# DhruvDh/highway-rope-ppo

Hardware: AMD Instinct MI355X
Metric: env-steps/sec (rollout+PPO update), 4096 envs × 15 vehicles, 1/2/4/8 GPUs (higher is better)
Workload: dtype fp32; 1 GPU; configs[1]: 4096 lockstep envs/GPU x 51 simulated vehicles, 15 observed x 4 features, sorted, no PE; PPO h256, 8 epochs x 32 minibatches (batch_size 64 -> 2048/64), rollout 32 steps/env; order=sorted, pe=none, obs_vehicles=15, envs_per_gpu=4096, global_envs=4096, rollout_len=32, samples_per_update=131072, hidden_dim=256, epochs=8, minibatches_per_epoch=32, parallelism=env-sharded dp1, library_build_flags=0

## Files before the change

### highway-rope-ppo_amd/csrc/ppo_kernels.hip

```cpp
#include <hip/hip_runtime.h>
#include <stdint.h>
#include <stdlib.h>
#include <string.h>

#include <algorithm>
#include <cmath>
#include <type_traits>

#include "hwy_ppo.h"

typedef float f32x16 __attribute__((ext_vector_type(16)));

#if defined(HWY_SECTION_PROFILE) || defined(HWY_CLOCK_PROBE)
__device__ unsigned long long g_ppo_sections[16];
#endif
#ifdef HWY_CLOCK_PROBE
__device__ unsigned long long g_ppo_wgt[2][1024][3];
#define CLK_BEGIN                                         \
  const uint64_t _c0 = __builtin_amdgcn_s_memtime();      \
  const uint64_t _r0 = __builtin_amdgcn_s_memrealtime();
#define CLK_END(k)                                                                   \
  do {                                                                               \
    if (threadIdx.x == 0) {                                                          \
      const uint64_t _r1 = __builtin_amdgcn_s_memrealtime();                         \
// ... 1139 lines not shown
    row_epi_bias_relu(acc, bias[0], H1, PH, nb);
  __syncthreads();
  if (h1g) rows_out<NT, RT>(H1, PH, h1g + (long)row0 * H, H, H, nrows);
  PSEC(1);
  zero_acc(acc);
  R.template run<1>(H1, PH, acc);
  if constexpr (MSK)
    mb[1] = row_epi_bias_relu_bits(acc, bias[1], H2, PH, nb);
  else
    row_epi_bias_relu(acc, bias[1], H2, PH, nb);
  __syncthreads();
  if (h2g) rows_out<NT, RT>(H2, PH, h2g + (long)row0 * H, H, H, nrows);
  PSEC(2);
  if constexpr (KEEP) {
    zero_acc(av);
    R.template run<2>(H2, PH, av);
    bias_relu_regs(av, bias[2]);
    zero_acc(cv);
    R.template run<3>(H2, PH, cv);
    bias_relu_regs(cv, bias[3]);
    return;
  }
  zero_acc(acc);
  R.template run<2>(H2, PH, acc);
  row_epi_bias_relu(acc, bias[2], AC, PA, nb);
  zero_acc(acc);
  R.template run<3>(H2, PH, acc);
  row_epi_bias_relu(acc, bias[3], AC + H, PA, nb);
  __syncthreads();
}

__device__ __forceinline__ float squash_corr(float z) {
  return log1pf(-(tanhf(z) * tanhf(z)) + 1e-6f);
}

template <int QH, int NW, int RT, bool CMP, bool WIDE = false>
__device__ __forceinline__ void rows_body(const RowArgs& r) {
  constexpr int H = 64 * QH;
  constexpr int TW = H / NW / 16;
  constexpr int RB = RT / 16;
  constexpr int RPW = RT / NW;
  constexpr int NT = 64 * NW;
  static_assert(TW * 16 * NW == H, "H must split into 16-column tiles per wave");
  static_assert(RT % 16 == 0 && RPW >= 1 && RPW <= 16, "RT: whole 16-row blocks, <= 16 head rows per wave");
  constexpr int PH = lds_pitch(H), PA = lds_pitch(2 * H), PXMAX = lds_pitch(kMaxRowS);
  constexpr bool kOwnX = !CMP && PXMAX > PA;
  static_assert(!CMP || (PA <= 2 * PH && PXMAX <= PH), "CMP: dac spans P0 | P1, the states fit P1");
  __shared__ __attribute__((aligned(16))) float XX[kOwnX ? RT * PXMAX : 4];
  __shared__ __attribute__((aligned(16))) float H1[CMP ? 2 * RT * PH : RT * PH];
  __shared__ __attribute__((aligned(16))) float H2[CMP ? 4 : RT * PH];
  __shared__ __attribute__((aligned(16))) float ACI[CMP ? 4 : RT * PA];
  float* const P1 = CMP ? H1 + RT * PH : H2;
  float* const AC = CMP ? H1 : ACI;
  __shared__ __attribute__((aligned(16))) f32x4 HDOT[NW][RT];
  __shared__ __attribute__((aligned(16))) f32x4 HROW[RT];
  __shared__ float HTAIL[NW][12];
#include "ppo_rows_body.inc"
}

template <int QH, int NW, int RT>
constexpr int rows_lds_floats() {
  constexpr int H = 64 * QH, PH = lds_pitch(H), PA = lds_pitch(2 * H), PXMAX = lds_pitch(kMaxRowS);
  return (PXMAX > PA ? RT * PXMAX : 0) + 2 * RT * PH + RT * PA + 4 * NW * RT + 4 * RT + 12 * NW;
}

template <int QH, int NW, int RT, bool WIDE = false>
__device__ __forceinline__ void rows_body_dyn(const RowArgs& r, float* arena) {
  constexpr bool CMP = false;
  constexpr int H = 64 * QH;
  constexpr int TW = H / NW / 16;
  constexpr int RB = RT / 16;
  constexpr int RPW = RT / NW;
  constexpr int NT = 64 * NW;
  static_assert(TW * 16 * NW == H && RT % 16 == 0 && RPW >= 1 && RPW <= 16, "rows_body's geometry");
  constexpr int PH = lds_pitch(H), PA = lds_pitch(2 * H), PXMAX = lds_pitch(kMaxRowS);
  constexpr bool kOwnX = PXMAX > PA;
  constexpr int oH1 = kOwnX ? RT * PXMAX : 0, oH2 = oH1 + RT * PH, oAC = oH2 + RT * PH;
  constexpr int oHD = oAC + RT * PA, oHR = oHD + 4 * NW * RT, oHT = oHR + 4 * RT;
  static_assert(oHT + 12 * NW == rows_lds_floats<QH, NW, RT>(), "arena layout");
  float* const XX = arena;
  float* const H1 = arena + oH1;
  float* const H2 = arena + oH2;
  float* const ACI = arena + oAC;
  float* const P1 = H2;
  float* const AC = ACI;
  f32x4(*const HDOT)[RT] = reinterpret_cast<f32x4(*)[RT]>(arena + oHD);
  f32x4* const HROW = reinterpret_cast<f32x4*>(arena + oHR);
  float(*const HTAIL)[12] = reinterpret_cast<float(*)[12]>(arena + oHT);
#include "ppo_rows_body.inc"
}

template <int QH, int NW, int RT>
__global__ void __launch_bounds__(64 * NW, 1) ppo_rows(RowArgs r) {
  rows_body<QH, NW, RT, false>(r);
}

template <int QH, int NW, int RT>
__global__ void __launch_bounds__(64 * NW) __attribute__((amdgpu_waves_per_eu(2 * NW / 4, 8)))
ppo_rows_c(RowArgs r) {
  CLK_BEGIN
  rows_body<QH, NW, RT, true>(r);
  CLK_END(0);
}

template <int QH, int NW>
__global__ void __launch_bounds__(64 * NW) __attribute__((amdgpu_waves_per_eu(NW / 4, 8)))
ppo_rows_c64(RowArgs r) {
  CLK_BEGIN
  rows_body<QH, NW, 64, true>(r);
  CLK_END(0);
}

struct ActArgs {
  int B, S;
  const float* states;
  const float* params;
  int64_t off[13];
  const float* noise;
  float *action, *pre_tanh, *logp, *value;
  const float* tiles;
#ifdef HWY_PPO_VMASK_TU
  const uint8_t *vm_trunc, *vm_term;
#endif
};

#ifdef HWY_PPO_VMASK_TU
__device__ __forceinline__ uint64_t vmask_tile(const ActArgs& r, int row0, int nrows, int lane) {
  bool mk = false;
  if (lane < nrows) {
    const long b = row0 + lane;
    mk = r.vm_trunc[b] != 0 && !(r.vm_term && r.vm_term[b] != 0);
  }
  return __ballot(mk);
}
#endif

template <int QH, int NW, bool TL, bool WIDE = false>
__device__ __forceinline__ void act_body(ActArgs r) {
  constexpr int H = 64 * QH;
  constexpr int RPW = kRowTile / NW;
  constexpr int PH = lds_pitch(H), PA = lds_pitch(2 * H), PXMAX = lds_pitch(kMaxRowS);
  __shared__ __attribute__((aligned(16))) float X[kRowTile * PXMAX];
  __shared__ __attribute__((aligned(16))) float H1[kRowTile * PH];
  __shared__ __attribute__((aligned(16))) float H2[kRowTile * PH];
  __shared__ __attribute__((aligned(16))) float AC[kRowTile * PA];
#include "ppo_act_body.inc"
}

template <int QH>
constexpr int act_lds_floats() {
  return kRowTile * (lds_pitch(kMaxRowS) + 2 * lds_pitch(64 * QH) + lds_pitch(128 * QH));
}
template <int QH, int NW, int RT>
constexpr int act_c_lds_floats() { return 2 * RT * lds_pitch(64 * QH) + 4 * NW * RT; }

template <int QH, int NW, bool TL, bool WIDE = false>
__device__ __forceinline__ void act_body_dyn(ActArgs r, float* arena) {
  constexpr int H = 64 * QH;
  constexpr int RPW = kRowTile / NW;
  constexpr int PH = lds_pitch(H), PA = lds_pitch(2 * H), PXMAX = lds_pitch(kMaxRowS);
  static_assert(kRowTile * (PXMAX + 2 * PH + PA) == act_lds_floats<QH>(), "arena layout");
  float* const X = arena;
  float* const H1 = arena + kRowTile * PXMAX;
  float* const H2 = arena + kRowTile * (PXMAX + PH);
  float* const AC = arena + kRowTile * (PXMAX + 2 * PH);
#include "ppo_act_body.inc"
}

template <int QH, int NW, bool TL>
__global__ void __launch_bounds__(64 * NW, 1) ppo_act(ActArgs r) {
  act_body<QH, NW, TL>(r);
}

template <int QH, int NW, int RT, bool WIDE = false>
__device__ __forceinline__ void act_c_body(ActArgs r) {
  constexpr int H = 64 * QH;
  constexpr int TW = H / NW / 16;
  constexpr int RB = RT / 16;
  constexpr int RPW = RT / NW;
  constexpr int PH = lds_pitch(H), PXMAX = lds_pitch(kMaxRowS);
  static_assert(TW * 16 * NW == H && PXMAX <= PH && RPW >= 1 && RPW <= 16, "ppo_act_c geometry");
  __shared__ __attribute__((aligned(16))) float P01[2 * RT * PH];
  __shared__ __attribute__((aligned(16))) f32x4 HDOT[NW][RT];
#include "ppo_act_c_body.inc"
}

template <int QH, int NW, int RT, bool WIDE = false>
__device__ __forceinline__ void act_c_body_dyn(ActArgs r, float* arena) {
  constexpr int H = 64 * QH;
  constexpr int TW = H / NW / 16;
  constexpr int RB = RT / 16;
  constexpr int RPW = RT / NW;
  constexpr int PH = lds_pitch(H), PXMAX = lds_pitch(kMaxRowS);
  static_assert(TW * 16 * NW == H && PXMAX <= PH && RPW >= 1 && RPW <= 16, "ppo_act_c geometry");
  static_assert(2 * RT * PH + 4 * NW * RT == act_c_lds_floats<QH, NW, RT>(), "arena layout");
  float* const P01 = arena;
  f32x4(*const HDOT)[RT] = reinterpret_cast<f32x4(*)[RT]>(arena + 2 * RT * PH);
#include "ppo_act_c_body.inc"
}

template <int QH, int NW, int RT>
__global__ void __launch_bounds__(64 * NW) __attribute__((amdgpu_waves_per_eu(2 * NW / 4, 8)))
ppo_act_c(ActArgs r) {
  act_c_body<QH, NW, RT>(r);
}

struct WgArgs {
  int B, S, H;
  const float *dac, *h2, *dh2, *h1, *dh1, *xg;
  float* grads;
  int64_t off[13];
  const float* head_part;
  int nhp, HP;
  float* norm_part;
  int tac, t2, t1, nh;
  int split;
  int bal, wm, tpe, nslot;
  float* slab;
  float entropy_coef, value_coef, ent_const;
  const float* params;
  float* metrics;
  int32_t* counters;
};

template <int NW = 4>
__device__ __forceinline__ float block_sum4(float v, float* red) {
  const int t = threadIdx.x;
  v = wave_sum_dpp(v);
  __syncthreads();
  if ((t & 63) == 0) red[t >> 6] = v;
  __syncthreads();
  float s = red[0];
#pragma unroll
  for (int i = 1; i < NW; ++i) s += red[i];
  return s;
}

__device__ void wgrad_head(const WgArgs& a, int hid, float* lds, float* red) {
  float(*tile)[64] = reinterpret_cast<float(*)[64]>(lds);
  const int t = threadIdx.x, lane = t & 63, w = t >> 6, H = a.H;
  const int e = hid * 64 + lane;
  const int ne = 3 * H + 9;
  const int per = (a.nhp + kWgWaves - 1) / kWgWaves, p0 = w * per, p1 = min(a.nhp, p0 + per);
  float s = 0.0f, sq = 0.0f;
  if (e < ne) {
    for (int pb = p0; pb < p1; pb += 16) {
      float pv[16];
#pragma unroll
      for (int u = 0; u < 16; ++u)
        pv[u] = pb + u < p1 ? a.head_part[(long)(pb + u) * a.HP + e] : 0.0f;
#pragma unroll
      for (int u = 0; u < 16; ++u) s += pv[u];
    }
  }
  tile[w][lane] = s;
  __syncthreads();
  if (t < 64 && e < ne) {
    float g = tile[0][t];
#pragma unroll
    for (int i = 1; i < kWgWaves; ++i) g += tile[i][t];
    long dst = -1;
    float gv = g;
    if (e < 2 * H) {
      dst = a.off[P_WA2] + e;
    } else if (e < 3 * H) {
      dst = a.off[P_WC2] + (e - 2 * H);
    } else {
      const int k = e - 3 * H;
      if (k < 2) dst = a.off[P_BA2] + k;
      else if (k == 2) dst = a.off[P_BC2];
      else if (k < 5) dst = a.off[P_LOGSTD] + (k - 3), gv = g - a.entropy_coef;
    }
    if (dst >= 0) {
      a.grads[dst] = gv;
      sq = gv * gv;
    }
    tile[0][t] = g;
  }
  const float tot = block_sum4<kWgWaves>(sq, red);
  if (t == 0) a.norm_part[hid] = tot;
  if (3 * H >= e - lane && 3 * H < e - lane + 64 && t == 0) {
    const int k0 = 3 * H - (e - lane);
    const float pg = tile[0][k0 + 5], vf = tile[0][k0 + 6], clip = tile[0][k0 + 7],
                kl = tile[0][k0 + 8];
    const float invB = 1.0f / (float)a.B;
    const float ls0 = a.params[a.off[P_LOGSTD]], ls1 = a.params[a.off[P_LOGSTD] + 1];
    const float ent = (a.ent_const + logf(expf(ls0))) + (a.ent_const + logf(expf(ls1)));
    float* m = a.metrics + (int64_t)(a.counters[1] - 1) * 6;
    m[0] = pg * invB;
    m[1] = vf * invB;
    m[2] = ent;
    m[3] = (pg * invB + a.value_coef * (vf * invB)) - a.entropy_coef * ent;
    m[4] = clip;
    m[5] = kl * invB;
  }
}

#define WG_ST(p, v) (*(p) = (v))

typedef __attribute__((address_space(3))) void lds_void_t;

__device__ __forceinline__ void wgrad_tile_dma(const WgArgs& a, int tile_id, int kb0, int kb1,
                                               float* part, float* wg_lds PSEC_PARAMS) {
  const int t = threadIdx.x, lane = t & 63, w = t >> 6, h = lane >> 5, l32 = lane & 31;
  const int H = a.H;
  if (kb1 <= kb0) {
    for (int i = t; i < kWgPart; i += 64 * kWgWaves) part[i] = 0.0f;
    return;
  }
  int id = tile_id;
  const float *A, *Bm;
  int lda, ldb, M, N, ntj;
  if (id < a.tac) {
    A = a.dac, lda = 2 * H, Bm = a.h2, ldb = H, M = 2 * H, N = H;
  } else if (id < a.tac + a.t2) {
    id -= a.tac;
    A = a.dh2, lda = H, Bm = a.h1, ldb = H, M = H, N = H;
  } else {
    id -= a.tac + a.t2;
    A = a.dh1, lda = H, Bm = a.xg, ldb = a.S, M = H, N = a.S;
  }
  ntj = (N + kWgTN - 1) / kWgTN;
  const int ti = id / ntj, tj = id % ntj;
  const int i0 = ti * kWgTM, j0 = tj * kWgTN;
  const int nchunk = (kb1 - kb0 + 63) / 64;
  constexpr int BUF = (kWgTM + kWgTN) * 64;

  const int rb = lane >> 4, qb = lane & 15;
  const uint32_t a_col = (uint32_t)min(i0 + 4 * (h ? ((l32 - 8) & 31) : l32), M - 4);
  const uint32_t b_col = (uint32_t)min(j0 + 4 * ((rb & 1) ? ((qb - 8) & 15) : qb), N - 4);
  auto dma = [&](int c, float* buf, int part = -1) {
    const int k0 = kb0 + 64 * c;
#pragma unroll
    for (int i = 0; i < 4; ++i) {
      if (part >= 0 && part != i / 2) continue;
      const uint32_t row = (uint32_t)min(k0 + 2 * (4 * w + i) + h, kb1 - 1);
      __builtin_amdgcn_global_load_lds((const void*)(A + (row * (uint32_t)lda + a_col)),
                                       (lds_void_t*)(buf + (4 * w + i) * 256), 16, 0, 0);
    }
#pragma unroll
    for (int i = 0; i < 2; ++i) {
      if (part >= 0 && part != 2) continue;
      const uint32_t row = (uint32_t)min(k0 + 4 * (2 * w + i) + rb, kb1 - 1);
      __builtin_amdgcn_global_load_lds((const void*)(Bm + (row * (uint32_t)ldb + b_col)),
                                       (lds_void_t*)(buf + kWgTM * 64 + (2 * w + i) * 256), 16,
                                       0, 0);
    }
  };
  const int kh = w >> 2, wq = w & 3;
  const int wm = (wq & 1) * 64, wn = (wq >> 1) * 32;
  const int offa0 = h * 128 + ((wm + l32 + 32 * h) & 127);
  const int offa1 = h * 128 + ((wm + 32 + l32 + 32 * h) & 127);
  const int offb = kWgTM * 64 + h * 64 + ((wn + l32 + 32 * h) & 63);
  f32x16 acc0, acc1;
#pragma unroll
  for (int q = 0; q < 16; ++q) acc0[q] = acc1[q] = 0.0f;
  float bs0 = 0.0f, bs1 = 0.0f;
  auto compute = [&](const float* buf, int lim, auto mask_tag, int dc, float* dbuf) {
    constexpr bool MASK = decltype(mask_tag)::value;
    const float* pa0 = buf + offa0 + 32 * kh * 128;
    const float* pa1 = buf + offa1 + 32 * kh * 128;
    const float* pb = buf + offb + 32 * kh * 64;
    float x0[2][4], x1[2][4], y[2][4];
    auto rd = [&](int g, int b) {
#pragma unroll
      for (int j = 0; j < 4; ++j) {
        const int st = 4 * g + j;
        x0[b][j] = pa0[st * 256];
        x1[b][j] = pa1[st * 256];
        y[b][j] = pb[st * 128];
      }
    };
    rd(0, 0);
#pragma unroll
    for (int g = 0; g < 4; ++g) {
      const int b = g & 1;
      if (g + 1 < 4) rd(g + 1, b ^ 1);
      __builtin_amdgcn_sched_barrier(0);
#pragma unroll
      for (int j = 0; j < 4; ++j) {
        float u0 = x0[b][j], u1 = x1[b][j];
        if constexpr (MASK) {
          const bool live = 32 * kh + 2 * (4 * g + j) + h < lim;
          u0 = live ? u0 : 0.0f;
          u1 = live ? u1 : 0.0f;
        }
        bs0 += u0;
        bs1 += u1;
        acc0 = __builtin_amdgcn_mfma_f32_32x32x2f32(u0, y[b][j], acc0, 0, 0, 0);
        acc1 = __builtin_amdgcn_mfma_f32_32x32x2f32(u1, y[b][j], acc1, 0, 0, 0);
      }
      __builtin_amdgcn_sched_barrier(0);
      if (g < 3 && dc >= 0) {
        dma(dc, dbuf, g);
        __builtin_amdgcn_sched_barrier(0);
      }
    }
  };
  const std::integral_constant<bool, true> masked;
  const std::integral_constant<bool, false> unmasked;
  float* b0 = wg_lds;
  float* b1 = wg_lds + BUF;
  float* b2 = wg_lds + 2 * BUF;
  asm volatile("s_waitcnt vmcnt(0)" ::: "memory");
  dma(0, b0);
  if (nchunk > 1) dma(1, b1);
  auto step = [&](int c, auto mask_tag) {
    if (c + 1 < nchunk)
      asm volatile("s_waitcnt vmcnt(6)" ::: "memory");
    else
      asm volatile("s_waitcnt vmcnt(0)" ::: "memory");
    asm volatile("s_waitcnt lgkmcnt(0)" ::: "memory");
    __builtin_amdgcn_s_barrier();
    compute(b0, kb1 - (kb0 + 64 * c), mask_tag, c + 2 < nchunk ? c + 2 : -1, b2);
    float* tb = b0;
    b0 = b1, b1 = b2, b2 = tb;
  };
  const int nfull = (kb1 - kb0) / 64;
  for (int c = 0; c < nfull; ++c) step(c, unmasked);
  if (nfull < nchunk) step(nfull, masked);
  asm volatile("s_waitcnt lgkmcnt(0)" ::: "memory");
  __builtin_amdgcn_s_barrier();
  PSEC(8);
  bs0 += __shfl_xor(bs0, 32);
  bs1 += __shfl_xor(bs1, 32);
  float* xch = wg_lds;
  float* bx = wg_lds + 4 * 32 * 64;
  if (kh == 1) {
#pragma unroll
    for (int q = 0; q < 16; ++q) {
      xch[(wq * 32 + q) * 64 + lane] = acc0[q];
      xch[(wq * 32 + 16 + q) * 64 + lane] = acc1[q];
    }
    if (h == 0) {
      bx[(wq * 2) * 32 + l32] = bs0;
      bx[(wq * 2 + 1) * 32 + l32] = bs1;
    }
  }
  __syncthreads();
  if (kh == 0) {
#pragma unroll
    for (int q = 0; q < 16; ++q) {
      const int ri = wm + (q & 3) + 8 * (q >> 2) + 4 * h;
      WG_ST(&part[ri * kWgTN + wn + l32], acc0[q] + xch[(wq * 32 + q) * 64 + lane]);
      WG_ST(&part[(ri + 32) * kWgTN + wn + l32], acc1[q] + xch[(wq * 32 + 16 + q) * 64 + lane]);
    }
    if (tj == 0 && wn == 0 && h == 0) {
      WG_ST(&part[kWgTM * kWgTN + wm + l32], bs0 + bx[(wq * 2) * 32 + l32]);
      WG_ST(&part[kWgTM * kWgTN + wm + 32 + l32], bs1 + bx[(wq * 2 + 1) * 32 + l32]);
    }
  }
  PSEC(9);
}

#define WGRAD_TILE wgrad_tile_dma

__device__ __forceinline__ void ppo_wgrad_body(const WgArgs& a) {
  PSEC_DECL
  constexpr int kWgBufs = 3;
  __shared__ __attribute__((aligned(16))) float wg_lds[kWgBufs * (kWgTM + kWgTN) * 64 + kWgWaves + 2];
  float* red = wg_lds + kWgBufs * (kWgTM + kWgTN) * 64;
  const int ntile = a.tac + a.t2 + a.t1;
  const int id = blockIdx.x;
  const int rows = (a.B + a.split - 1) / a.split;
  if (!a.bal) {
    if (id >= ntile * a.split) {
      wgrad_head(a, id - ntile * a.split, wg_lds, red);
      PSEC(10);
      PSEC_FLUSH;
      return;
    }
    const int z = id % a.split, tile = id / a.split;
    const int kb0 = z * rows, kb1 = min(a.B, kb0 + rows);
    WGRAD_TILE(a, tile, kb0, kb1, a.slab + ((long)tile * a.split + z) * kWgPart,
               wg_lds PSEC_ARGS);
    PSEC_FLUSH;
    return;
  }
  const int z = id % a.split, j = id / a.split;
  const int kz = min(a.B, z * rows), kz1 = min(a.B, kz + rows), km = min(kz1, kz + 64 * a.wm);
  auto slot = [&](int tile, int sl) {
    return a.slab + (((long)tile * a.split + z) * a.nslot + sl) * kWgPart;
  };
  if (j < ntile) {
    WGRAD_TILE(a, j, kz, km, slot(j, 0), wg_lds PSEC_ARGS);
  } else {
    const int e = j - ntile, nextra = (int)gridDim.x / a.split - ntile;
    const int t0 = min(ntile, e * a.tpe), t1 = min(ntile, t0 + a.tpe);
    for (int tile = t0; tile < t1; ++tile) {
      if (tile > t0) __syncthreads();
      WGRAD_TILE(a, tile, km, kz1, slot(tile, 1), wg_lds PSEC_ARGS);
    }
    if (e == nextra - 1) {
      for (int hid = z; hid < a.nh; hid += a.split) {
        __syncthreads();
        wgrad_head(a, hid, wg_lds, red);
      }
      PSEC(10);
    }
  }
  PSEC_FLUSH;
}

__global__ void __launch_bounds__(512) ppo_wgrad(WgArgs a) {
  CLK_BEGIN
  ppo_wgrad_body(a);
  CLK_END(1);
}

__device__ __forceinline__ float wsum_item(const WgArgs& a, int item) {
  const int t = threadIdx.x, H = a.H;
  constexpr int kParts = kWgTM * kWgTN / 1024;
  const int tile_id = item / kParts, part = item % kParts;
  int id = tile_id, M, N, region;
  if (id < a.tac) {
    M = 2 * H, N = H, region = 0;
  } else if (id < a.tac + a.t2) {
    id -= a.tac, M = H, N = H, region = 1;
  } else {
    id -= a.tac + a.t2, M = H, N = a.S, region = 2;
  }
  const int ntj = (N + kWgTN - 1) / kWgTN;
  const int ti = id / ntj, tj = id % ntj, i0 = ti * kWgTM, j0 = tj * kWgTN;
  auto grad_row = [&](int i) -> long {
    if (region == 0) return i < H ? a.off[P_WA1] + (long)i * H : a.off[P_WC1] + (long)(i - H) * H;
    if (region == 1) return a.off[P_W2] + (long)i * H;
    return a.off[P_W1] + (long)i * a.S;
  };
  const float* sl = a.slab + (long)tile_id * a.split * a.nslot * kWgPart;
  const int e = part * 1024 + 4 * t, ri = e / kWgTN, cj = e % kWgTN;
  constexpr int kMaxParts = 16;
  const int np = a.split * a.nslot;
  f32x4 pv[kMaxParts];
#pragma unroll
  for (int q = 0; q < kMaxParts; ++q)
    if (q < np) pv[q] = *reinterpret_cast<const f32x4*>(sl + (long)q * kWgPart + e);
  const bool bias_t = part == 0 && tj == 0 && t < kWgTM && i0 + t < M;
  float bp[kMaxParts];
#pragma unroll
  for (int q = 0; q < kMaxParts; ++q)
    bp[q] = (bias_t && q < np) ? sl[(long)q * kWgPart + kWgTM * kWgTN + t] : 0.0f;
  f32x4 v = pv[0];
#pragma unroll
  for (int q = 1; q < kMaxParts; ++q)
    if (q < np) v += pv[q];
  float sq = 0.0f;
  if (i0 + ri < M) {
    const long row = grad_row(i0 + ri) + j0 + cj;
    float* dst = a.grads + row;
#pragma unroll
    for (int c4 = 0; c4 < 4; ++c4)
      if (j0 + cj + c4 < N) {
        dst[c4] = v[c4];
        sq += v[c4] * v[c4];
      }
  }
  if (bias_t) {
    float b = 0.0f;
#pragma unroll
    for (int q = 0; q < kMaxParts; ++q)
      if (q < np) b += bp[q];
    const int i = i0 + t;
    long bo;
    if (region == 0) bo = i < H ? a.off[P_BA1] + i : a.off[P_BC1] + (i - H);
    else if (region == 1) bo = a.off[P_B2] + i;
    else bo = a.off[P_B1] + i;
    a.grads[bo] = b;
    sq += b * b;
  }
  return sq;
}

__device__ __forceinline__ void wsum_body(const WgArgs& a) {
  __shared__ float red[4];
  const float tot = block_sum4(wsum_item(a, blockIdx.x), red);
  if (threadIdx.x == 0) a.norm_part[a.nh + blockIdx.x] = tot;
}

__global__ void __launch_bounds__(256) ppo_wsum(WgArgs a) { wsum_body(a); }

struct RedDesc {
  const float* src;
  int64_t stride;
  int32_t nsplit;
  int64_t numel;
  int64_t dst;
};
struct RedArgs {
  RedDesc d[13];
  float* grads;
  float* norm_part;
  int64_t numel;
  const float* head_tail;
  int HP, nhead, B;
  float value_coef, entropy_coef, ent_const;
  const float* params;
  int64_t off_ls;
  float* metrics;
  int32_t* counters;
};

__global__ void __launch_bounds__(kRedThreads) ppo_reduce(RedArgs r) {
  __shared__ float red[kRedThreads / 64];
  const int64_t i = (int64_t)blockIdx.x * kRedThreads + threadIdx.x;
  float sq = 0.0f;
  if (i < r.numel) {
    int p = 0;
#pragma unroll 1
    for (int q = 1; q < 13; ++q)
      if (i >= r.d[q].dst) p = q;
    const RedDesc& D = r.d[p];
    const int64_t j = i - D.dst;
    float s = 0.0f;
#pragma unroll 8
    for (int z = 0; z < D.nsplit; ++z) s += D.src[z * D.stride + j];
    if (p == P_LOGSTD) s = s - r.entropy_coef;
    r.grads[i] = s;
    sq = s * s;
  }
  sq = wave_sum_dpp(sq);
  if ((threadIdx.x & 63) == 0) red[threadIdx.x >> 6] = sq;
  __syncthreads();
  if (threadIdx.x == 0) {
    float s = 0.0f;
    for (int k = 0; k < kRedThreads / 64; ++k) s += red[k];
    r.norm_part[blockIdx.x] = s;
  }
  if (blockIdx.x == 0 && threadIdx.x == 0) {
    float pg = 0.0f, vf = 0.0f, clip = 0.0f, kl = 0.0f;
#pragma unroll 8
    for (int z = 0; z < r.nhead; ++z) {
      const float* tl = r.head_tail + (int64_t)z * r.HP;
      pg += tl[5];
      vf += tl[6];
      clip += tl[7];
      kl += tl[8];
    }
    const float invB = 1.0f / (float)r.B;
    const float ls0 = r.params[r.off_ls], ls1 = r.params[r.off_ls + 1];
    const float ent = (r.ent_const + logf(expf(ls0))) + (r.ent_const + logf(expf(ls1)));
    float* m = r.metrics + (int64_t)(r.counters[1] - 1) * 6;
    m[0] = pg * invB;
    m[1] = vf * invB;
    m[2] = ent;
    m[3] = (pg * invB + r.value_coef * (vf * invB)) - r.entropy_coef * ent;
    m[4] = clip;
    m[5] = kl * invB;
  }
}

struct OptArgs {
  float* params;
  const float* grads;
  float* m;
  float* v;
  const float* norm_part;
  int nred;
  int64_t numel;
  const int32_t* counters;
  float lr, beta1, beta2, eps, max_norm;
  float* tiles;
  int64_t o_w1, o_w2, o_wa1, o_wc1;
  int S, H, sb, hb;
  int skip;
  int nwg1, nwgh, nkg1;
  int64_t run_off[4], run_pre[5];
};

__device__ __forceinline__ int64_t tile_index(int k, int n, int nblk) {
  return ((int64_t)(n >> 4) * nblk + (k >> 4)) * 256 + ((((k & 15) >> 2) << 4) + (n & 15)) * 4 +
         (k & 3);
}

__device__ __forceinline__ void write_tiles(const OptArgs& o, int64_t i, float v) {
  const TileGeom T = tile_geom(o.S, o.H, o.sb, o.hb);
  const int64_t H = o.H;
  int64_t j = i - o.o_w1;
  if (j >= 0 && j < H * o.S) {
    const int n = (int)(((float)j + 0.5f) * (1.0f / (float)o.S));
    const int k = (int)(j - (int64_t)n * o.S);
    o.tiles[T.f1 + tile_index(k, n, o.sb)] = v;
    return;
  }
  const int64_t offs[3] = {o.o_w2, o.o_wa1, o.o_wc1};
  const int64_t fwd[3] = {T.f2, T.fa, T.fc}, bwd[3] = {T.b2, T.ba, T.bc};
#pragma unroll
  for (int q = 0; q < 3; ++q) {
    j = i - offs[q];
    if (j >= 0 && j < H * H) {
      const int n = (int)(((float)j + 0.5f) * (1.0f / (float)o.H));
      const int k = (int)(j - (int64_t)n * H);
      o.tiles[fwd[q] + tile_index(k, n, o.hb)] = v;
      o.tiles[bwd[q] + tile_index(n, k, o.hb)] = v;
      return;
    }
  }
}

struct TileArgs {
  const float* P;
  int64_t o_w1, o_w2, o_wa1, o_wc1;
  int S, H, sb, hb;
  float* tiles;
};

__global__ void __launch_bounds__(256) ppo_retile(TileArgs a) {
  const TileGeom T = tile_geom(a.S, a.H, a.sb, a.hb);
  const int64_t i = (int64_t)blockIdx.x * 256 + threadIdx.x;
  if (i >= T.total) return;
  const float* W;
  int64_t base;
  int K, nblk;
  bool fwd;
  if (i < T.f2) W = a.P + a.o_w1, base = T.f1, K = a.S, nblk = a.sb, fwd = true;
  else if (i < T.fa) W = a.P + a.o_w2, base = T.f2, K = a.H, nblk = a.hb, fwd = true;
  else if (i < T.fc) W = a.P + a.o_wa1, base = T.fa, K = a.H, nblk = a.hb, fwd = true;
  else if (i < T.ba) W = a.P + a.o_wc1, base = T.fc, K = a.H, nblk = a.hb, fwd = true;
  else if (i < T.bc) W = a.P + a.o_wa1, base = T.ba, K = a.H, nblk = a.hb, fwd = false;
  else if (i < T.b2) W = a.P + a.o_wc1, base = T.bc, K = a.H, nblk = a.hb, fwd = false;
  else W = a.P + a.o_w2, base = T.b2, K = a.H, nblk = a.hb, fwd = false;
  const int64_t r = i - base;
  const int tile = (int)(r >> 8), e = (int)(r & 255);
  const int G = tile / nblk, b = tile - G * nblk;
// ... 1715 lines not shown
```

Before: 6.053 million env-steps/s.

## Stagger k-halves of wgrad tile kernel across chunks with lean DMA addressing

Restructures the weight-gradient tile loop so the upper k-half waves (kh=1) run half a chunk out of phase with the lower half, raised to higher priority with s_setprio. Interior chunks use a precomputed, unclamped base-plus-offset DMA address path, and only the last chunks keep the clamped path. LDS reads for the next group are moved to the middle of the MFMA group. The aim is to spread LDS and DMA traffic across the two wave groups and cut per-chunk address arithmetic. The cost is much more complex barrier and wait choreography, which risks ordering bugs and extra synchronisation waits.

```diff
diff --git a/highway-rope-ppo_amd/csrc/ppo_kernels.hip b/highway-rope-ppo_amd/csrc/ppo_kernels.hip
--- a/highway-rope-ppo_amd/csrc/ppo_kernels.hip
+++ b/highway-rope-ppo_amd/csrc/ppo_kernels.hip
@@ -1465,7 +1465,8 @@
 
 __device__ __forceinline__ void wgrad_tile_dma(const WgArgs& a, int tile_id, int kb0, int kb1,
                                                float* part, float* wg_lds PSEC_PARAMS) {
-  const int t = threadIdx.x, lane = t & 63, w = t >> 6, h = lane >> 5, l32 = lane & 31;
+  const int t = threadIdx.x, lane = t & 63, h = lane >> 5, l32 = lane & 31;
+  const int w = __builtin_amdgcn_readfirstlane(t >> 6);
   const int H = a.H;
   if (kb1 <= kb0) {
     for (int i = t; i < kWgPart; i += 64 * kWgWaves) part[i] = 0.0f;
@@ -1510,6 +1511,28 @@
                                        0, 0);
     }
   };
+  const char* ga = (const char*)(A + (size_t)(kb0 + 128 + 8 * w) * (size_t)lda);
+  const char* gb = (const char*)(Bm + (size_t)(kb0 + 128 + 8 * w) * (size_t)ldb);
+  uint32_t la[4], lb[2];
+#pragma unroll
+  for (int i = 0; i < 4; ++i) la[i] = ((uint32_t)((2 * i + h) * lda) + a_col) * 4u;
+#pragma unroll
+  for (int i = 0; i < 2; ++i) lb[i] = ((uint32_t)((4 * i + rb) * ldb) + b_col) * 4u;
+  auto dma_whole = [&](float* buf, int part) {
+#pragma unroll
+    for (int i = 0; i < 4; ++i) {
+      if (part != i / 2) continue;
+      __builtin_amdgcn_global_load_lds((const void*)(ga + la[i]),
+                                       (lds_void_t*)(buf + (4 * w + i) * 256), 16, 0, 0);
+    }
+#pragma unroll
+    for (int i = 0; i < 2; ++i) {
+      if (part != 2) continue;
+      __builtin_amdgcn_global_load_lds((const void*)(gb + lb[i]),
+                                       (lds_void_t*)(buf + kWgTM * 64 + (2 * w + i) * 256), 16,
+                                       0, 0);
+    }
+  };
   const int kh = w >> 2, wq = w & 3;
   const int wm = (wq & 1) * 64, wn = (wq >> 1) * 32;
   const int offa0 = h * 128 + ((wm + l32 + 32 * h) & 127);
@@ -1519,8 +1542,10 @@
 #pragma unroll
   for (int q = 0; q < 16; ++q) acc0[q] = acc1[q] = 0.0f;
   float bs0 = 0.0f, bs1 = 0.0f;
-  auto compute = [&](const float* buf, int lim, auto mask_tag, int dc, float* dbuf) {
+  auto compute = [&](const float* buf, int lim, auto mask_tag, auto dma_tag, int dc,
+                     float* dbuf) {
     constexpr bool MASK = decltype(mask_tag)::value;
+    constexpr int DMA = decltype(dma_tag)::value;
     const float* pa0 = buf + offa0 + 32 * kh * 128;
     const float* pa1 = buf + offa1 + 32 * kh * 128;
     const float* pb = buf + offb + 32 * kh * 64;
@@ -1538,10 +1563,13 @@
 #pragma unroll
     for (int g = 0; g < 4; ++g) {
       const int b = g & 1;
-      if (g + 1 < 4) rd(g + 1, b ^ 1);
       __builtin_amdgcn_sched_barrier(0);
 #pragma unroll
       for (int j = 0; j < 4; ++j) {
+        if (j == 2) {
+          if (g + 1 < 4) rd(g + 1, b ^ 1);
+          __builtin_amdgcn_sched_barrier(0);
+        }
         float u0 = x0[b][j], u1 = x1[b][j];
         if constexpr (MASK) {
           const bool live = 32 * kh + 2 * (4 * g + j) + h < lim;
@@ -1554,7 +1582,11 @@
         acc1 = __builtin_amdgcn_mfma_f32_32x32x2f32(u1, y[b][j], acc1, 0, 0, 0);
       }
       __builtin_amdgcn_sched_barrier(0);
-      if (g < 3 && dc >= 0) {
+      if (g < 3 && DMA == 1) {
+        dma_whole(dbuf, g);
+        __builtin_amdgcn_sched_barrier(0);
+      }
+      if (g < 3 && DMA == 2 && dc >= 0) {
         dma(dc, dbuf, g);
         __builtin_amdgcn_sched_barrier(0);
       }
@@ -1566,22 +1598,117 @@
   float* b1 = wg_lds + BUF;
   float* b2 = wg_lds + 2 * BUF;
   asm volatile("s_waitcnt vmcnt(0)" ::: "memory");
+  if (kh) __builtin_amdgcn_s_setprio(1);
   dma(0, b0);
-  if (nchunk > 1) dma(1, b1);
-  auto step = [&](int c, auto mask_tag) {
+  if (nchunk > 1 && !kh) dma(1, b1);
+  auto step = [&](int c, auto mask_tag, auto dma_tag) {
     if (c + 1 < nchunk)
       asm volatile("s_waitcnt vmcnt(6)" ::: "memory");
     else
       asm volatile("s_waitcnt vmcnt(0)" ::: "memory");
     asm volatile("s_waitcnt lgkmcnt(0)" ::: "memory");
     __builtin_amdgcn_s_barrier();
-    compute(b0, kb1 - (kb0 + 64 * c), mask_tag, c + 2 < nchunk ? c + 2 : -1, b2);
+    compute(b0, kb1 - (kb0 + 64 * c), mask_tag, dma_tag, c + 2 < nchunk ? c + 2 : -1, b2);
     float* tb = b0;
     b0 = b1, b1 = b2, b2 = tb;
+    if (decltype(dma_tag)::value == 1) ga += (size_t)lda * 256, gb += (size_t)ldb * 256;
   };
   const int nfull = (kb1 - kb0) / 64;
-  for (int c = 0; c < nfull; ++c) step(c, unmasked);
-  if (nfull < nchunk) step(nfull, masked);
+  const int nlean = max(nfull - 2, 0);
+  const std::integral_constant<int, 0> dma_none;
+  const std::integral_constant<int, 1> dma_lean;
+  const std::integral_constant<int, 2> dma_clamped;
+  auto run = [&]() {
+    for (int c = 0; c < nlean; ++c) step(c, unmasked, dma_lean);
+    for (int c = nlean; c < nfull; ++c) step(c, unmasked, dma_clamped);
+    if (nfull < nchunk) step(nfull, masked, dma_none);
+  };
+  float xs0[2][4], xs1[2][4], ys[2][4];
+  auto compute_st = [&](const float* bufp, const float* buf, int limp, int lim, auto mask_tag,
+                        auto dma_tag, auto half_tag, int dc, float* dbuf) {
+    constexpr bool MASK = decltype(mask_tag)::value;
+    constexpr int DMA = decltype(dma_tag)::value;
+    constexpr int HALF = decltype(half_tag)::value;
+    constexpr int K0 = HALF == 2 ? 2 : 0, K1 = HALF == 3 ? 2 : 4;
+    auto& x0 = xs0;
+    auto& x1 = xs1;
+    auto& y = ys;
+    auto rd = [&](int k, int b) {
+      const float* p = k < 2 ? bufp : buf;
+      const float* pa0 = p + offa0 + 32 * kh * 128;
+      const float* pa1 = p + offa1 + 32 * kh * 128;
+      const float* pb = p + offb + 32 * kh * 64;
+#pragma unroll
+      for (int j = 0; j < 4; ++j) {
+        const int st = 4 * ((k + 2) & 3) + j;
+        x0[b][j] = pa0[st * 256];
+        x1[b][j] = pa1[st * 256];
+        y[b][j] = pb[st * 128];
+      }
+    };
+    if (HALF == 2 && DMA == 2 && dc >= 0) dma(dc, dbuf);
+    if (HALF == 2) rd(2, 0);
+#pragma unroll
+    for (int k = K0; k < K1; ++k) {
+      const int b = k & 1, g = (k + 2) & 3, l = k < 2 ? limp : lim;
+      __builtin_amdgcn_sched_barrier(0);
+#pragma unroll
+      for (int j = 0; j < 4; ++j) {
+        if (j == 2) {
+          if (k + 1 < K1 || HALF != 3) rd(k + 1, b ^ 1);
+          __builtin_amdgcn_sched_barrier(0);
+        }
+        float u0 = x0[b][j], u1 = x1[b][j];
+        if constexpr (MASK) {
+          const bool live = 32 * kh + 2 * (4 * g + j) + h < l;
+          u0 = live ? u0 : 0.0f;
+          u1 = live ? u1 : 0.0f;
+        }
+        bs0 += u0;
+        bs1 += u1;
+        acc0 = __builtin_amdgcn_mfma_f32_32x32x2f32(u0, y[b][j], acc0, 0, 0, 0);
+        acc1 = __builtin_amdgcn_mfma_f32_32x32x2f32(u1, y[b][j], acc1, 0, 0, 0);
+      }
+      __builtin_amdgcn_sched_barrier(0);
+      if (HALF == 1 && k < 3 && DMA == 1) {
+        dma_whole(dbuf, k);
+        __builtin_amdgcn_sched_barrier(0);
+      }
+      if (HALF == 1 && k < 3 && DMA == 2 && dc >= 0) {
+        dma(dc, dbuf, k);
+        __builtin_amdgcn_sched_barrier(0);
+      }
+    }
+  };
+  auto step_st = [&](int c, auto mask_tag, auto dma_tag, auto half_tag) {
+    asm volatile("s_waitcnt vmcnt(0)" ::: "memory");
+    asm volatile("s_waitcnt lgkmcnt(0)" ::: "memory");
+    __builtin_amdgcn_s_barrier();
+    const int lim = kb1 - (kb0 + 64 * c);
+    compute_st(b2, b0, lim + 64, lim, mask_tag, dma_tag, half_tag, c + 1 < nchunk ? c + 1 : -1,
+               b1);
+    float* tb = b0;
+    b0 = b1, b1 = b2, b2 = tb;
+    if (decltype(dma_tag)::value == 1) ga += (size_t)lda * 256, gb += (size_t)ldb * 256;
+  };
+  const std::integral_constant<int, 1> both;
+  const std::integral_constant<int, 2> head;
+  const std::integral_constant<int, 3> tail;
+  auto run_st = [&]() {
+    step_st(0, masked, dma_clamped, head);
+    for (int c = 1; c < 1 + nlean; ++c) step_st(c, unmasked, dma_lean, both);
+    for (int c = 1 + nlean; c < nfull; ++c) step_st(c, unmasked, dma_clamped, both);
+    if (nfull < nchunk && nfull >= 1) step_st(nfull, masked, dma_none, both);
+    step_st(nchunk, masked, dma_none, tail);
+  };
+  if (kh) {
+    run_st();
+    __builtin_amdgcn_s_setprio(0);
+  } else {
+    run();
+    asm volatile("s_waitcnt lgkmcnt(0)" ::: "memory");
+    __builtin_amdgcn_s_barrier();
+  }
   asm volatile("s_waitcnt lgkmcnt(0)" ::: "memory");
   __builtin_amdgcn_s_barrier();
   PSEC(8);
```

Result: faster. 6.126 million env-steps/s (median of 6 runs) (+1.2%).
